# csmile-1006/ARP

Measured on AMD Instinct MI355X. Metric: frames/sec CLIP reward-labelled (256x256 ViT-B/32), higher is better.
Workload: dtype f16; 1 GPU; CLIP ViT-B/32 reward labelling, batch 1024 synthetic 256x256x3 uint8 frames per GPU resident in HBM (BASELINE.json configs[1]), random-init weights, text tower cached; parallelism=shard1 (no collective), streams_per_gpu=2

## Files before the change

### arp_amd/csrc/gemm.h

```cpp
#pragma once
#include "common.h"

#ifndef ARP_ADAMW_PIPE
#define ARP_ADAMW_PIPE 1
#endif
namespace arp {

struct GemmArgs {
    const void* A = nullptr;
    const void* W = nullptr;
    const float* bias = nullptr;
    const float* resid = nullptr;
    void* out = nullptr;
    int M = 0, N = 0, K = 0;
    int lda = 0, ldw = 0, ldr = 0, ldo = 0;
    int flags = 0;
    unsigned long long* clock_acc = nullptr;
    int ksplit = 1;
    size_t slice_stride = 0;
    const float* ln_stats = nullptr;
    const float* ln_c = nullptr;
    int ln_parts = 0;
    float ln_inv_d = 0.f, ln_eps = 0.f;
    void* xb_out = nullptr;
    int ldxb = 0;
    int m_fast = 0;
    int split3 = 0;
    float* stats_out = nullptr;
    int group_m = 0;
    int stagger_groups = 0;
    int stagger_cycles = 0;
    float alpha = 1.f;
    float out_scale = 1.f;
    const void* mask = nullptr;
    int ldm = 0;
    float* colsum_part = nullptr;
    int ovl = 0;
    float *adam_p = nullptr, *adam_m = nullptr, *adam_v = nullptr;
    void* adam_mirror = nullptr;
    int adam_mask = 0;
    unsigned int* adam_dropped = nullptr;
    float adam_gscale = 1.f, adam_lr = 0.f, adam_wd = 0.f, adam_b1 = 0.f, adam_b2 = 0.f, adam_eps = 0.f, adam_bc1 = 1.f, adam_bc2 = 1.f;
    int mix_nk16 = 0, mix_nkc_a = 0, mix_sa = 0, mix_sb = 0;
    int x8_shift = -1;
    void* dx4_out = nullptr;
    const int* mix_sptr = nullptr;
};
constexpr int GEMM_SITE_ADAMW = 26;

template <typename OutT>
inline int gemm_epilogue_refusal(const GemmArgs& g, bool fp4_side, const char* who) {
    const bool staged = ((g.N | g.ldo | g.ldr) & 3) == 0 && ((g.N | g.ldo) & (sizeof(OutT) == 1 ? 15 : 7)) == 0 && !(g.flags & 2);
    const bool fp4 = g.x8_shift >= 0 || g.dx4_out;
    const std::string w(who);
    if ((g.ln_stats || g.xb_out || g.stats_out || fp4) && !staged)
        return fail(w + ": the folded LayerNorm and the side outputs need the staged epilogue (N, ldo % 8 == 0; ldr % 4 == 0)");
    if (g.ln_stats && sizeof(OutT) != 2) return fail(w + ": the folded-LayerNorm consumer has a 16-bit output");
    if ((g.stats_out || g.split3) && sizeof(OutT) != 4) return fail(w + ": stats_out / split3 belong to the f32 epilogue");
    if (g.stats_out && g.N % 128) return fail(w + ": stats_out needs N % 128 == 0 (one (sum, sum of squares) pair per 128 columns)");
    if (fp4 && !fp4_side) return fail(w + ": the fp4 side outputs exist on the MIXC binary16-output instances only");
    if ((g.x8_shift >= 0 && !g.xb_out) || (g.split3 && !g.xb_out)) return fail(w + ": x8_shift / split3 without xb_out");
    if (g.xb_out && sizeof(OutT) != 4 && g.x8_shift < 0) return fail(w + ": xb_out of a 16-bit output is the x4 segment (x8_shift >= 0)");
    return 0;
}

constexpr int GEMM_BM = 128, GEMM_BN = 128, GEMM_THREADS = 256;
constexpr int GEMM_ROW_BYTES = 128;
constexpr int GEMM_STAGE_BYTES = (GEMM_BM + GEMM_BN) * GEMM_ROW_BYTES;
constexpr int GEMM_LDS_BYTES = 2 * GEMM_STAGE_BYTES;

__device__ __forceinline__ int xcd_remap(int bid, int nwg) {
    const int q = nwg >> 3, r = nwg & 7, xcd = bid & 7;
    const int base = (xcd < r) ? xcd * (q + 1) : r * (q + 1) + (xcd - r) * q;
    return base + (bid >> 3);
}

__device__ __forceinline__ void ln_row_stats(const GemmArgs& g, int m, float& mu, float& rs) {
    const float* st = g.ln_stats + (size_t)m * g.ln_parts * 2;
    float s = 0.f, q = 0.f;
    for (int p = 0; p < g.ln_parts; ++p) {
        s += st[2 * p];
        q += st[2 * p + 1];
    }
    mu = s * g.ln_inv_d;
    rs = 1.0f / sqrtf(fmaxf(q * g.ln_inv_d - mu * mu, 0.f) + g.ln_eps);
}
__device__ __forceinline__ float half_wave_sum(float v) {
#pragma unroll
    for (int o = 16; o > 0; o >>= 1) v += __shfl_xor(v, o, 64);
    return v;
}

template <typename T, typename OutT, int ACT, bool RESID, int SITE, int STAGES = 2>
__global__ __launch_bounds__(GEMM_THREADS) void gemm_nt_kernel(GemmArgs g) {
    extern __shared__ __attribute__((aligned(16))) char smem[];
    constexpr int EPB = GEMM_ROW_BYTES / (int)sizeof(T);
    constexpr int EPC = 16 / (int)sizeof(T);

    const int tid = threadIdx.x;
    const int lane = tid & 63;
    const int wave = __builtin_amdgcn_readfirstlane(tid >> 6);
    const int n_tiles = (g.N + GEMM_BN - 1) / GEMM_BN;
    const int m_tiles = (g.M + GEMM_BM - 1) / GEMM_BM;
    const int tile = xcd_remap(blockIdx.x, m_tiles * n_tiles);
    const int m0 = (g.m_fast ? tile % m_tiles : tile / n_tiles) * GEMM_BM;
    const int n0 = (g.m_fast ? tile / m_tiles : tile % n_tiles) * GEMM_BN;

    const T* __restrict__ A = static_cast<const T*>(g.A);
    const T* __restrict__ W = static_cast<const T*>(g.W);

    if (g.stagger_groups > 1 && blockIdx.x >= 256 && blockIdx.x < 512 && blockIdx.y == 0) {
        const unsigned long long t0 = __builtin_amdgcn_s_memtime();
        while (__builtin_amdgcn_s_memtime() - t0 < (unsigned long long)g.stagger_cycles) __builtin_amdgcn_s_sleep(64);
    }

    const int srow = lane >> 3;
    const int schunk = (lane & 7) ^ srow;
    const T* a_src[4];
    const T* w_src[4];
#pragma unroll
// ... 328 lines not shown
```

### arp_amd/csrc/gemm256.h

```cpp
#pragma once
#include <cstdlib>
#include <type_traits>

#include "common.h"
#include "gemm.h"

namespace arp {

#ifndef ARP_G2_TWO_PHASE
#define ARP_G2_TWO_PHASE 1
#endif
#ifndef ARP_G2_OVERLAP_DRAIN
#define ARP_G2_OVERLAP_DRAIN 0
#endif
constexpr int G2_BM = 256, G2_BN = 256, G2_THREADS = 512;
constexpr int G2_BUF_BYTES = (G2_BM + G2_BN) * 128;
static_assert(256 * (256 * 2 + 16) >= 2 * G2_BUF_BYTES && 256 * (256 * 2 + 16) >= 128 * (256 * 4 + 16), "epilogue tile must cover the K-tile ring");
constexpr int G2_TILE_BYTES = 256 * (256 * 2 + 16);
constexpr bool G2_MASK_SITE(int site) { return site >= 16; }
constexpr int G2_RED_OFF = G2_TILE_BYTES + 1024;
constexpr int G2_LDS_BYTES = G2_RED_OFF + 8 * 256 * 4;
constexpr int G2_B_REGION = G2_BM * 128;
constexpr int G2_GROUP_M = 8;

template <int N> __device__ __forceinline__ void wait_vmcnt() {
    if constexpr (N == 0) asm volatile("s_waitcnt vmcnt(0)" ::: "memory");
    if constexpr (N == 2) asm volatile("s_waitcnt vmcnt(2)" ::: "memory");
    if constexpr (N == 4) asm volatile("s_waitcnt vmcnt(4)" ::: "memory");
    if constexpr (N == 6) asm volatile("s_waitcnt vmcnt(6)" ::: "memory");
    if constexpr (N == 8) asm volatile("s_waitcnt vmcnt(8)" ::: "memory");
    if constexpr (N == 24) asm volatile("s_waitcnt vmcnt(24)" ::: "memory");
}
__device__ __forceinline__ void wait_units(int allow) {
    if (allow >= 3) wait_vmcnt<6>();
    else if (allow == 2) wait_vmcnt<4>();
    else if (allow == 1) wait_vmcnt<2>();
    else wait_vmcnt<0>();
}

#if defined(ARP_G2_STAMPS) || defined(ARP_G2_FINE) || defined(ARP_G2_CLOCK)
__device__ long long* arp_g2_stamps = nullptr;
#endif
#ifndef ARP_G2_MAX_VGPR
#define ARP_G2_MAX_VGPR 128
#endif
#ifndef ARP_G2_MFMA32
#define ARP_G2_MFMA32 0
#endif
#ifndef ARP_G2_MIXC_RT
#define ARP_G2_MIXC_RT 0
#endif
#ifndef ARP_G2_MIX_UNIFORM
#define ARP_G2_MIX_UNIFORM 0
#endif
#ifndef ARP_G2_ABL
#define ARP_G2_ABL 0
#endif
typedef __attribute__((ext_vector_type(16))) float f32x16_v;
template <typename T> __device__ __forceinline__ f32x16_v mfma32(u32x4_v a, u32x4_v b, f32x16_v c) {
    if constexpr (__is_same(T, f16_t))
        return __builtin_amdgcn_mfma_f32_32x32x16_f16(__builtin_bit_cast(f16x8_v, a), __builtin_bit_cast(f16x8_v, b), c, 0, 0, 0);
    else
        return __builtin_amdgcn_mfma_f32_32x32x16_bf16(__builtin_bit_cast(bf16x8_v, a), __builtin_bit_cast(bf16x8_v, b), c, 0, 0, 0);
}
template <typename T, typename OutT, int ACT, bool RESID, int SITE, bool M32 = (ARP_G2_MFMA32 != 0), int KV = ARP_G2_KV, bool MIXC = false, bool CLK = false>
__global__ __launch_bounds__(G2_THREADS, 2) __attribute__((amdgpu_num_vgpr(ARP_G2_MAX_VGPR))) void gemm256_nt_kernel(GemmArgs g) {
    extern __shared__ __attribute__((aligned(16))) char smem[];
    constexpr int EPB = 128 / (int)sizeof(T);
    constexpr int EPC = 16 / (int)sizeof(T);
    constexpr bool W32 = M32 && sizeof(T) == 2;

    const int tid = threadIdx.x;
    const int lane = tid & 63;
    const int wave = __builtin_amdgcn_readfirstlane(tid >> 6);
    const int wr = wave >> 2, wc = wave & 3;
#ifdef ARP_G2_CLOCK
    const long long clk_c0 = __builtin_amdgcn_s_memtime(), clk_r0 = __builtin_amdgcn_s_memrealtime();
#endif
    [[maybe_unused]] unsigned long long dclk_c0 = 0, dclk_r0 = 0;
    if constexpr (CLK) {
        dclk_c0 = __builtin_amdgcn_s_memtime();
        dclk_r0 = __builtin_amdgcn_s_memrealtime();
        __builtin_amdgcn_s_waitcnt(0xC07F);
    }

    const int n_tiles = (g.N + G2_BN - 1) / G2_BN;
    const int m_tiles = (g.M + G2_BM - 1) / G2_BM;
    const int total_tiles = m_tiles * n_tiles;
    const int group_m = g.group_m > 0 ? g.group_m : G2_GROUP_M;
    int m0 = 0, n0 = 0;
    auto tile_coords = [&](int tix) __attribute__((always_inline)) {
        int t = xcd_remap(tix, total_tiles);
        const int per_group = group_m * n_tiles;
        const int grp = t / per_group;
        const int first_m = grp * group_m;
        const int gsize = min(m_tiles - first_m, group_m);
// ... 189 lines not shown
    int mix_scale = 0;
    int mix_sa = g.mix_sa, mix_sb = g.mix_sb;
    if constexpr (MIXC) {
        if (g.mix_sptr) {
            mix_sa = F16C_X_SHIFT + g.mix_sptr[0];
            mix_sb = F16C_DX_SHIFT + g.mix_sptr[1];
        }
    }
    auto mfma_quadrant = [&](auto MQ, auto NQ, auto F8 = F16T{}) __attribute__((always_inline)) {
        constexpr int mq = decltype(MQ)::value, nq = decltype(NQ)::value;
        if constexpr (MIXC && sizeof(T) == 2 && !W32) {
            if constexpr (decltype(F8)::value) {
#pragma unroll
                for (int ks = 0; ks < 2; ++ks)
#pragma unroll
                    for (int ni = 0; ni < 2; ++ni)
#pragma unroll
                        for (int mi = 0; mi < 4; ++mi) acc[mq][nq][ni][mi] = mfma_fp4_scaled(breg[nq][ni][ks], areg[mi][ks], acc[mq][nq][ni][mi], mix_scale);
                return;
            }
        }
        if constexpr (W32) {
#pragma unroll
            for (int ks = 0; ks < 4; ++ks)
#pragma unroll
                for (int mi = 0; mi < 2; ++mi) acc32[mq][nq][mi] = mfma32<T>(breg[nq][0][ks], areg[mi][ks], acc32[mq][nq][mi]);
        } else {
#pragma unroll
        for (int ks = 0; ks < 2; ++ks)
#pragma unroll
            for (int ni = 0; ni < 2; ++ni)
#pragma unroll
                for (int mi = 0; mi < 4; ++mi) {
                    if constexpr (sizeof(T) == 2) {
                        acc[mq][nq][ni][mi] = mfma16<T>(breg[nq][ni][ks], areg[mi][ks], acc[mq][nq][ni][mi]);
                    } else if constexpr (sizeof(T) == 1) {
                        if (ks == 0)
                            acc[mq][nq][ni][mi] = mfma_fp8(breg[nq][ni][0], breg[nq][ni][1], areg[mi][0], areg[mi][1], acc[mq][nq][ni][mi]);
                    } else {
#pragma unroll
                        for (int j = 0; j < 4; ++j)
                            acc[mq][nq][ni][mi] = __builtin_amdgcn_mfma_f32_16x16x4f32(
                                __uint_as_float(breg[nq][ni][ks][j]), __uint_as_float(areg[mi][ks][j]), acc[mq][nq][ni][mi], 0, 0, 0);
                    }
                }
        }
    };
    auto phase_tail = [&](int ph) __attribute__((always_inline)) {
        int allow = G - 3 - ph;
        allow = allow > 3 ? 3 : allow;
        wait_units(allow);
        __builtin_amdgcn_sched_barrier(0);
        __builtin_amdgcn_s_barrier();
        __builtin_amdgcn_sched_barrier(0);
    };
    auto compute = [&](auto MQ, auto NQ) __attribute__((always_inline)) {
        __builtin_amdgcn_s_setprio(1);
        mfma_quadrant(MQ, NQ);
        __builtin_amdgcn_s_setprio(0);
        __builtin_amdgcn_sched_barrier(0);
        __builtin_amdgcn_s_barrier();
        __builtin_amdgcn_sched_barrier(0);
    };
#if ARP_G2_TWO_PHASE
    const int S2 = 2 * nk;
    auto issue_step = [&](int st) __attribute__((always_inline)) {
        const int t4 = (st >> 1) * 4;
        if (st & 1) {
            issue(t4 + 3, U3{});
        } else {
            issue(t4 + 0, U0{});
            issue(t4 + 1, U1{});
            issue(t4 + 2, U2{});
        }
    };
    auto step_cnt = [&](int st) __attribute__((always_inline)) { return st < S2 ? ((st & 1) ? 2 : 6) : 0; };
    auto wait_instr = [&](int n) __attribute__((always_inline)) {
        if (n >= 24) wait_vmcnt<24>();
        else if (n >= 8) wait_vmcnt<8>();
        else if (n >= 6) wait_vmcnt<6>();
        else if (n >= 2) wait_vmcnt<2>();
        else wait_vmcnt<0>();
    };
    int young = 0;
    auto phase_tail2 = [&](int p) __attribute__((always_inline)) {
        wait_instr(step_cnt(p + 2) + step_cnt(p + 3) + (p + 1 <= 2 ? young : 0));
        asm volatile("s_waitcnt lgkmcnt(0)" ::: "memory");
        __builtin_amdgcn_sched_barrier(0);
        __builtin_amdgcn_s_barrier();
        __builtin_amdgcn_sched_barrier(0);
    };
    auto compute2 = [&](auto MQ, auto NQA, auto NQB, auto F8 = F16T{}) __attribute__((always_inline)) {
        __builtin_amdgcn_s_setprio(1);
        mfma_quadrant(MQ, NQA, F8);
        mfma_quadrant(MQ, NQB, F8);
        __builtin_amdgcn_s_setprio(0);
        __builtin_amdgcn_sched_barrier(0);
        __builtin_amdgcn_s_barrier();
        __builtin_amdgcn_sched_barrier(0);
    };
#endif
    bool pre_issued = false;
    bool pre_issued_bias = false;
    bool pre4 = false;
    for (int tix = blockIdx.x; tix < total_tiles; tix += gridDim.x) {
#ifdef ARP_G2_STAMPS
    long long st_[6];
    st_[0] = __builtin_amdgcn_s_memtime();
#define ARP_STAMP(i) st_[i] = __builtin_amdgcn_s_memtime()
#else
#define ARP_STAMP(i)
#endif
    tile_coords(tix);
    setup_src();
    float* bias_s = reinterpret_cast<float*>(smem + G2_TILE_BYTES);
    if (g.bias && wave == 0 && !pre_issued_bias) bias_dma(n0);
    if constexpr (W32) {
#pragma unroll
        for (int a = 0; a < 2; ++a)
#pragma unroll
            for (int b = 0; b < 2; ++b)
#pragma unroll
                for (int c = 0; c < 2; ++c)
#pragma unroll
                    for (int d = 0; d < 16; ++d) acc32[a][b][c][d] = 0.f;
    } else {
#pragma unroll
    for (int a = 0; a < 2; ++a)
#pragma unroll
        for (int b = 0; b < 2; ++b)
#pragma unroll
            for (int c = 0; c < 2; ++c)
#pragma unroll
                for (int d = 0; d < 4; ++d) acc[a][b][c][d] = f32x4_v{0.f, 0.f, 0.f, 0.f};
    }
#ifdef ARP_G2_FINE
    long long f_[12];
    for (int i = 0; i < 12; ++i) f_[i] = 0;
#define ARP_FST(i) if (kt == (nk >> 1)) f_[i] = __builtin_amdgcn_s_memtime()
#else
#define ARP_FST(i)
#endif
#if ARP_G2_TWO_PHASE
    if (!pre_issued) {
        issue_step(0);
        issue_step(1);
        issue_step(2);
    }
    young = pre4 ? 16 : 0;
    wait_instr(step_cnt(1) + step_cnt(2) + young);
    __builtin_amdgcn_sched_barrier(0);
    __builtin_amdgcn_s_barrier();
    __builtin_amdgcn_sched_barrier(0);
    if (wr == 1) {
        __builtin_amdgcn_s_barrier();
    }
    __builtin_amdgcn_sched_barrier(0);

    int kt_first = 0;
    if constexpr (KV == 1 && !ARP_G2_OVERLAP_DRAIN) {
        auto tail_ss = [&]() __attribute__((always_inline)) {
            wait_vmcnt<8>();
            __builtin_amdgcn_s_waitcnt(0xC07F);
            __builtin_amdgcn_sched_barrier(0);
            __builtin_amdgcn_s_barrier();
            __builtin_amdgcn_sched_barrier(0);
        };
        auto ktile_ss = [&](int kt, auto BUF, auto F8) __attribute__((always_inline)) {
            const char* buf = smem + ((MIXC && RESID && ARP_G2_MIXC_RT) ? (kt & 1) : decltype(BUF)::value) * G2_BUF_BYTES;
            if constexpr (MIXC && decltype(F8)::value) mix_scale = 0x7f7f7f00 | (127 - (kt < g.mix_nk16 + g.mix_nkc_a ? mix_sa : mix_sb));
            load_a(buf, 0, F8);
            load_b(buf, I0{}, F8);
            load_b(buf, I1{}, F8);
            issue_ss(kt + 1, U3{});
            tail_ss();
            compute2(I0{}, I0{}, I1{}, F8);
            load_a(buf, 1, F8);
            issue_ss(kt + 2, U0{});
            issue_ss(kt + 2, U1{});
            issue_ss(kt + 2, U2{});
            tail_ss();
            compute2(I1{}, I1{}, I0{}, F8);
        };
        auto run_ss = [&](int kt_end, auto F8) __attribute__((always_inline)) {
            if (kt_first < kt_end && (kt_first & 1)) {
                ktile_ss(kt_first, I1{}, F8);
                ++kt_first;
            }
            for (; kt_first + 1 < kt_end; kt_first += 2) {
                ktile_ss(kt_first, I0{}, F8);
                ktile_ss(kt_first + 1, I1{}, F8);
            }
            if (kt_first < kt_end) {
                ktile_ss(kt_first, I0{}, F8);
                ++kt_first;
            }
        };
        if constexpr (MIXC) {
            run_ss(g.mix_nk16, F16T{});
            run_ss(nk, F8T{});
            kt_first = nk;
        } else {
            run_ss(nk - 2, F16T{});
        }
    }
    auto ktile_tail = [&](int kt, auto F8) __attribute__((always_inline)) {
        const char* buf = smem + (kt & 1) * G2_BUF_BYTES;
        const int p = 2 * kt;
        abl_kt = kt;
        if constexpr (MIXC && decltype(F8)::value) mix_scale = 0x7f7f7f00 | (127 - (kt < g.mix_nk16 + g.mix_nkc_a ? mix_sa : mix_sb));
        ARP_FST(0);
        load_a(buf, 0, F8);
        load_b(buf, I0{}, F8);
        load_b(buf, I1{}, F8);
        issue_step(p + 3);
        ARP_FST(1);
        phase_tail2(p);
        ARP_FST(2);
        compute2(I0{}, I0{}, I1{}, F8);
        ARP_FST(4);
        load_a(buf, 1, F8);
        issue_step(p + 4);
        ARP_FST(5);
        phase_tail2(p + 1);
        ARP_FST(6);
        compute2(I1{}, I1{}, I0{}, F8);
        ARP_FST(8);
    };
    if constexpr (!MIXC) {
        for (int kt = kt_first; kt < nk; ++kt) ktile_tail(kt, F16T{});
    }
    if constexpr (MIXC) wait_vmcnt<0>();
#else
    if (!pre_issued) {
        issue(0, U0{});
        issue(1, U1{});
        issue(2, U2{});
        issue(3, U3{});
        issue(4, U0{});
    }
    {
        const int last = G - 1 < 4 ? G - 1 : 4;
        wait_units(last - 1);
// ... 22 lines not shown
        issue(ph + 7, U3{});
        phase_tail(ph + 2);
        compute(I1{}, I1{});
        issue(ph + 8, U0{});
        phase_tail(ph + 3);
        compute(I1{}, I0{});
    }
#endif
    if (wr == 0) {
        __builtin_amdgcn_s_barrier();
    }
    __builtin_amdgcn_sched_barrier(0);
    if constexpr (MIXC) {
        __builtin_amdgcn_s_barrier();
        __builtin_amdgcn_sched_barrier(0);
    }
#ifdef ARP_G2_FINE
    if (arp_g2_stamps && (threadIdx.x & 63) == 0) {
        long long* d = arp_g2_stamps + ((size_t)tix * 8 + wave) * 16;
        for (int i = 0; i < 9; ++i) d[i] = f_[i];
    }
#endif

    ARP_STAMP(1);
    auto epilogue = [&]() {
    OutT* out = static_cast<OutT*>(g.out);
#ifdef ARP_G2_EXPERIMENT_SAME_TILE
    if (g.flags & 16) out -= (size_t)m0 * g.ldo + n0;
#endif
    const bool vec_ok = ((g.N | g.ldo | g.ldr) & 3) == 0;
    if (g.flags & 1) {
        float sacc = 0.f;
#pragma unroll
        for (int a = 0; a < 2; ++a)
#pragma unroll
            for (int b = 0; b < 2; ++b)
#pragma unroll
                for (int c = 0; c < NI; ++c)
#pragma unroll
                    for (int d = 0; d < MI; ++d) {
                        const f32x4_v t = acc4(a, b, c, d);
                        sacc += t[0] + t[1] + t[2] + t[3];
                    }
        if (sacc == 12345.678f) Elem<OutT>::st(out, sacc);
        return;
    }
    const bool staged = vec_ok && ((g.N | g.ldo) & (sizeof(OutT) == 1 ? 15 : 7)) == 0 && !(g.flags & 2);
    if (staged) {
        float4 bq[2][NI];
#pragma unroll
        for (int nq = 0; nq < 2; ++nq)
#pragma unroll
            for (int ni = 0; ni < NI; ++ni)
                bq[nq][ni] = g.bias ? *reinterpret_cast<const float4*>(bias_s + wc * 64 + nq * 32 + ni * CSTEP + cl) : make_float4(0.f, 0.f, 0.f, 0.f);
        if constexpr (sizeof(OutT) == 1) {
            constexpr int RS8 = 256 + 16;
#pragma unroll
            for (int mq = 0; mq < 2; ++mq)
#pragma unroll
                for (int mi = 0; mi < MI; ++mi) {
                    const int row = wr * 128 + mq * 64 + mi * RSTEP + rl;
#pragma unroll
                    for (int nq = 0; nq < 2; ++nq)
#pragma unroll
                        for (int ni = 0; ni < NI; ++ni) {
                            const int col = wc * 64 + nq * 32 + ni * CSTEP + cl;
                            const f32x4_v a4 = acc4(mq, nq, ni, mi);
                            const float4 b = bq[nq][ni];
                            float v[4] = {a4[0] * g.alpha + b.x, a4[1] * g.alpha + b.y, a4[2] * g.alpha + b.z, a4[3] * g.alpha + b.w};
#pragma unroll
                            for (int j = 0; j < 4; ++j) v[j] = apply_act<ACT, true>(v[j]) * g.out_scale;
                            *reinterpret_cast<uint32_t*>(smem + row * RS8 + col) = pack_fp8x4(v[0], v[1], v[2], v[3]);
                        }
                }
            __syncthreads();
#pragma unroll 4
            for (int it = 0; it < 8; ++it) {
                const int r = it * 32 + wave * 4 + (lane >> 4);
                const int m = m0 + r, n = n0 + (lane & 15) * 16;
                if (m < g.M && n < g.N)
                    *reinterpret_cast<u32x4_v*>(reinterpret_cast<char*>(out) + (size_t)m * g.ldo + n) = *reinterpret_cast<const u32x4_v*>(smem + r * RS8 + (lane & 15) * 16);
            }
        } else if constexpr (sizeof(OutT) == 2) {
            constexpr int RS = 256 * 2 + 16;
            auto stage16 = [&](auto LN) {
                float* lnst = reinterpret_cast<float*>(smem + G2_RED_OFF);
                float4 cq[LN.value ? 2 : 1][LN.value ? NI : 1];
                if constexpr (LN.value) {
                    if (tid < 256) {
                        const float2* st = reinterpret_cast<const float2*>(g.ln_stats + (size_t)min(m0 + tid, g.M - 1) * g.ln_parts * 2);
                        float2 pr[8];
#pragma unroll
                        for (int p = 0; p < 8; ++p) pr[p] = st[min(p, g.ln_parts - 1)];
                        float s = 0.f, q = 0.f;
#pragma unroll
                        for (int p = 0; p < 8; ++p)
                            if (p < g.ln_parts) { s += pr[p].x; q += pr[p].y; }
                        const float mu = s * g.ln_inv_d;
                        lnst[2 * tid] = mu;
                        lnst[2 * tid + 1] = 1.0f / sqrtf(fmaxf(q * g.ln_inv_d - mu * mu, 0.f) + g.ln_eps);
                    }
#pragma unroll
                    for (int nq = 0; nq < 2; ++nq)
#pragma unroll
                        for (int ni = 0; ni < NI; ++ni)
                            cq[nq][ni] = *reinterpret_cast<const float4*>(g.ln_c + min(n0 + wc * 64 + nq * 32 + ni * CSTEP + cl, g.N - 4));
                    __syncthreads();
                }
#pragma unroll
                for (int mq = 0; mq < 2; ++mq)
#pragma unroll
                    for (int mi = 0; mi < MI; ++mi) {
                        const int row = wr * 128 + mq * 64 + mi * RSTEP + rl;
                        float mu = 0.f, rs = 1.f;
                        if constexpr (LN.value) { mu = lnst[2 * row]; rs = lnst[2 * row + 1]; }
#pragma unroll
                        for (int nq = 0; nq < 2; ++nq)
#pragma unroll
                            for (int ni = 0; ni < NI; ++ni) {
                                const int col = wc * 64 + nq * 32 + ni * CSTEP + cl;
                                const f32x4_v a4 = acc4(mq, nq, ni, mi);
                                float v[4] = {a4[0], a4[1], a4[2], a4[3]};
                                if constexpr (sizeof(T) == 1) { v[0] *= g.alpha; v[1] *= g.alpha; v[2] *= g.alpha; v[3] *= g.alpha; }
                                if constexpr (LN.value) {
                                    const float4 c4 = cq[LN.value ? nq : 0][LN.value ? ni : 0];
                                    v[0] = rs * (v[0] - mu * c4.x); v[1] = rs * (v[1] - mu * c4.y);
                                    v[2] = rs * (v[2] - mu * c4.z); v[3] = rs * (v[3] - mu * c4.w);
                                }
                                if constexpr ((ARP_G2_ABL & 8) == 0) {
                                    const float4 b = bq[nq][ni];
                                    v[0] += b.x; v[1] += b.y; v[2] += b.z; v[3] += b.w;
                                    apply_act4<ACT, sizeof(T) <= 2>(v);
                                }
                                *reinterpret_cast<uint2*>(smem + row * RS + col * 2) = make_uint2(pack2<OutT>(v[0], v[1]), pack2<OutT>(v[2], v[3]));
                                if constexpr (MIXC && __is_same(OutT, f16_t)) {
                                    if (g.dx4_out && m0 + row < g.M && n0 + col < g.N) {
                                        constexpr float sdx = (float)(1 << F16C_DX_SHIFT);
                                        *reinterpret_cast<uint16_t*>(static_cast<char*>(g.dx4_out) + (size_t)(m0 + row) * g.ldxb + ((n0 + col) >> 1)) =
                                            pack_fp4x4((v[0] - h2f(f2h(v[0]))) * sdx, (v[1] - h2f(f2h(v[1]))) * sdx, (v[2] - h2f(f2h(v[2]))) * sdx, (v[3] - h2f(f2h(v[3]))) * sdx);
                                    }
                                }
                            }
                    }
            };
            if constexpr (G2_MASK_SITE(SITE)) {
                stage16(std::false_type{});
            } else {
                if (g.ln_stats) stage16(std::true_type{});
                else stage16(std::false_type{});
            }
#if ARP_G2_TWO_PHASE && ARP_G2_OVERLAP_DRAIN
            if (g.ovl && tix + (int)gridDim.x < total_tiles && m0 + G2_BM <= g.M && n0 + G2_BN <= g.N && nk >= 4) {
                asm volatile("s_waitcnt lgkmcnt(0)" ::: "memory");
                __builtin_amdgcn_sched_barrier(0);
                __builtin_amdgcn_s_barrier();
                __builtin_amdgcn_sched_barrier(0);
                u32x4_v regs[16];
#pragma unroll
                for (int it = 0; it < 16; ++it)
                    regs[it] = *reinterpret_cast<const u32x4_v*>(smem + (it * 16 + wave * 2 + (lane >> 5)) * RS + (lane & 31) * 16);
                asm volatile("s_waitcnt lgkmcnt(0)" ::: "memory");
                __builtin_amdgcn_sched_barrier(0);
                __builtin_amdgcn_s_barrier();
                __builtin_amdgcn_sched_barrier(0);
                OutT* obase = out + (size_t)(m0 + wave * 2 + (lane >> 5)) * g.ldo + n0 + (lane & 31) * 8;
                tile_coords(tix + gridDim.x);
                setup_src();
                if (g.bias && wave == 0) bias_dma(n0);
                issue_step(0);
                issue_step(1);
                issue_step(2);
                __builtin_amdgcn_sched_barrier(0);
#pragma unroll
                for (int it = 0; it < 16; ++it) *reinterpret_cast<u32x4_v*>(obase + (size_t)it * 16 * g.ldo) = regs[it];
                __builtin_amdgcn_sched_barrier(0);
                pre_issued = pre_issued_bias = pre4 = true;
                return;
            }
#endif
            ARP_STAMP(2);
            __syncthreads();
            ARP_STAMP(3);
            if (G2_MASK_SITE(SITE) && g.mask) {
                const OutT* __restrict__ mk = static_cast<const OutT*>(g.mask);
                float colacc[8] = {0.f, 0.f, 0.f, 0.f, 0.f, 0.f, 0.f, 0.f};
#pragma unroll 4
                for (int it = 0; it < 16; ++it) {
                    const int r = it * 16 + wave * 2 + (lane >> 5);
                    const int m = m0 + r, n = n0 + (lane & 31) * 8;
                    if (m < g.M && n < g.N) {
                        u32x4_v v = *reinterpret_cast<const u32x4_v*>(smem + r * RS + (lane & 31) * 16);
                        const u32x4_v mv = *reinterpret_cast<const u32x4_v*>(mk + (size_t)m * g.ldm + n);
#pragma unroll
                        for (int w = 0; w < 4; ++w) {
                            const uint32_t mag = mv[w] & 0x7fff7fffu;
                            const uint32_t nz = ((mag & 0xffffu) ? 0xffffu : 0u) | ((mag >> 16) ? 0xffff0000u : 0u);
                            const uint32_t pos = ((mv[w] & 0x8000u) ? 0u : 0xffffu) | ((mv[w] & 0x80000000u) ? 0u : 0xffff0000u);
                            const uint32_t kept = v[w] & nz & pos;
                            v[w] = kept;
                            OutT pr[2];
                            memcpy(pr, &kept, 4);
                            colacc[2 * w] += Elem<OutT>::ld(&pr[0]);
                            colacc[2 * w + 1] += Elem<OutT>::ld(&pr[1]);
                        }
                        *reinterpret_cast<u32x4_v*>(out + (size_t)m * g.ldo + n) = v;
                    }
                }
                if (g.colsum_part) {
                    float* red = reinterpret_cast<float*>(smem + G2_RED_OFF);
#pragma unroll
                    for (int e = 0; e < 8; ++e) colacc[e] += __shfl_xor(colacc[e], 32, 64);
                    if (lane < 32) {
#pragma unroll
                        for (int e = 0; e < 8; ++e) red[wave * 256 + lane * 8 + e] = colacc[e];
                    }
                    __syncthreads();
                    if (tid < 256 && n0 + tid < g.N) {
                        float t = 0.f;
#pragma unroll
                        for (int w = 0; w < 8; ++w) t += red[w * 256 + tid];
                        g.colsum_part[(size_t)(m0 / G2_BM) * g.N + n0 + tid] = t;
                    }
                }
                return;
            }
#pragma unroll 4
            for (int it = 0; it < 16; ++it) {
                const int r = it * 16 + wave * 2 + (lane >> 5);
                const int m = m0 + r, n = n0 + (lane & 31) * 8;
                if (m < g.M && n < g.N) {
                    const u32x4_v v = *reinterpret_cast<const u32x4_v*>(smem + r * RS + (lane & 31) * 16);
                    if (g.flags & 4) __builtin_nontemporal_store(v, reinterpret_cast<u32x4_v*>(out + (size_t)m * g.ldo + n));
                    else *reinterpret_cast<u32x4_v*>(out + (size_t)m * g.ldo + n) = v;
                    if constexpr (MIXC && __is_same(OutT, f16_t)) {
                        if (g.x8_shift >= 0) {
                            const float inv = 1.0f / (float)(1 << g.x8_shift);
                            const uint32_t e0 = v[0], e1 = v[1], e2 = v[2], e3 = v[3];
                            uint32_t w4 = 0;
                            w4 = __builtin_amdgcn_cvt_scalef32_pk_fp4_f16(w4, __builtin_bit_cast(f16x2_v, e0), inv, 0);
                            w4 = __builtin_amdgcn_cvt_scalef32_pk_fp4_f16(w4, __builtin_bit_cast(f16x2_v, e1), inv, 1);
                            w4 = __builtin_amdgcn_cvt_scalef32_pk_fp4_f16(w4, __builtin_bit_cast(f16x2_v, e2), inv, 2);
                            w4 = __builtin_amdgcn_cvt_scalef32_pk_fp4_f16(w4, __builtin_bit_cast(f16x2_v, e3), inv, 3);
                            *reinterpret_cast<uint32_t*>(static_cast<char*>(g.xb_out) + (size_t)m * g.ldxb + (n >> 1)) = w4;
                        }
                    }
                }
            }
        } else {
            constexpr int RSF = 256 * 4 + 16;
#ifndef ARP_G2_RES_EARLY
#define ARP_G2_RES_EARLY 1
#endif
            float4 rres[2][16];
            auto load_res = [&](int p) {
                if constexpr (RESID) {
#pragma unroll
                    for (int it = 0; it < 16; ++it) {
                        const int lr = it * 8 + wave;
                        const int m = m0 + (lr >> 6) * 128 + p * 64 + (lr & 63), n = n0 + lane * 4;
                        if constexpr ((ARP_G2_ABL & 4) == 0) rres[p][it] = *reinterpret_cast<const float4*>(g.resid + (size_t)min(m, g.M - 1) * g.ldr + min(n, g.N - 4));
                        else rres[p][it] = make_float4(0.f, 0.f, 0.f, 0.f);
                    }
// ... 17 lines not shown
                            if constexpr (sizeof(T) == 1) { v[0] *= g.alpha; v[1] *= g.alpha; v[2] *= g.alpha; v[3] *= g.alpha; }
                            const float4 b = bq[nq][ni];
                            v[0] += b.x; v[1] += b.y; v[2] += b.z; v[3] += b.w;
#pragma unroll
                            for (int j = 0; j < 4; ++j) v[j] = apply_act<ACT, sizeof(T) <= 2>(v[j]);
                            *reinterpret_cast<float4*>(smem + lrow * RSF + col * 4) = make_float4(v[0], v[1], v[2], v[3]);
                        }
                __syncthreads();
                if (p == 0 && ARP_G2_RES_EARLY) load_res(1);
#pragma unroll
                for (int it = 0; it < 16; ++it) {
                    const int lr = it * 8 + wave;
                    const int m = m0 + (lr >> 6) * 128 + p * 64 + (lr & 63), n = n0 + lane * 4;
                    const bool ok = m < g.M && n < g.N;
                    float4 v = make_float4(0.f, 0.f, 0.f, 0.f);
                    if (ok) {
                        v = *reinterpret_cast<const float4*>(smem + lr * RSF + lane * 16);
                        if constexpr (RESID) {
                            const float4 r = rres[p][it];
                            v.x += r.x; v.y += r.y; v.z += r.z; v.w += r.w;
                        }
                        if (g.out) *reinterpret_cast<float4*>(reinterpret_cast<float*>(out) + (size_t)m * g.ldo + n) = v;
                        if (g.xb_out) {
                            if (g.split3) store_split3(static_cast<T*>(g.xb_out) + (size_t)m * g.ldxb + n, (size_t)g.N, v.x, v.y, v.z, v.w);
                            else store4(static_cast<T*>(g.xb_out) + (size_t)m * g.ldxb + n, v.x, v.y, v.z, v.w);
                        }
                    }
                    if (g.stats_out) {
                        const float s = half_wave_sum((v.x + v.y) + (v.z + v.w));
                        const float q = half_wave_sum((v.x * v.x + v.y * v.y) + (v.z * v.z + v.w * v.w));
                        if ((lane & 31) == 0 && ok) {
                            float* st = g.stats_out + ((size_t)m * (g.N >> 7) + ((n0 >> 7) + (lane >> 5))) * 2;
                            st[0] = s;
                            st[1] = q;
                        }
                    }
                }
            }
        }
        return;
    }
#pragma unroll
    for (int mq = 0; mq < 2; ++mq)
#pragma unroll
        for (int mi = 0; mi < MI; ++mi) {
            const int m = m0 + wr * 128 + mq * 64 + mi * RSTEP + rl;
            if (m >= g.M) continue;
#pragma unroll
            for (int nq = 0; nq < 2; ++nq)
#pragma unroll
                for (int ni = 0; ni < NI; ++ni) {
                    const int n = n0 + wc * 64 + nq * 32 + ni * CSTEP + cl;
                    if (n >= g.N) continue;
                    const f32x4_v a4 = acc4(mq, nq, ni, mi);
                    float v[4] = {a4[0], a4[1], a4[2], a4[3]};
                    if constexpr (sizeof(T) == 1) { v[0] *= g.alpha; v[1] *= g.alpha; v[2] *= g.alpha; v[3] *= g.alpha; }
                    if (vec_ok) {
                        if (g.bias) {
                            const float4 b = *reinterpret_cast<const float4*>(g.bias + n);
                            v[0] += b.x; v[1] += b.y; v[2] += b.z; v[3] += b.w;
                        }
#pragma unroll
                        for (int j = 0; j < 4; ++j) v[j] = apply_act<ACT, sizeof(T) <= 2>(v[j]);
                        if constexpr (RESID) {
                            const float4 r = *reinterpret_cast<const float4*>(g.resid + (size_t)m * g.ldr + n);
                            v[0] += r.x; v[1] += r.y; v[2] += r.z; v[3] += r.w;
                        }
                        store4(out + (size_t)m * g.ldo + n, v[0], v[1], v[2], v[3]);
                    } else {
#pragma unroll
                        for (int j = 0; j < 4; ++j) {
                            if (n + j >= g.N) break;
                            float x = v[j] + (g.bias ? g.bias[n + j] : 0.f);
                            x = apply_act<ACT, sizeof(T) <= 2>(x);
                            if constexpr (RESID) x += g.resid[(size_t)m * g.ldr + n + j];
                            Elem<OutT>::st(out + (size_t)m * g.ldo + n + j, x);
                        }
                    }
                }
        }
    };
    pre_issued = false;
    pre_issued_bias = false;
    pre4 = false;
    epilogue();
#ifdef ARP_G2_STAMPS
    ARP_STAMP(4);
    asm volatile("s_waitcnt vmcnt(0)" ::: "memory");
    ARP_STAMP(5);
    if (arp_g2_stamps && (threadIdx.x & 63) == 0) {
        long long* d = arp_g2_stamps + ((size_t)tix * 8 + wave) * 8;
        for (int i = 0; i < 6; ++i) d[i] = st_[i];
    }
#endif
    if (!pre_issued && tix + (int)gridDim.x < total_tiles) {
        __syncthreads();
        tile_coords(tix + gridDim.x);
        setup_src();
        if (g.bias && wave == 0) bias_dma(n0);
        pre_issued_bias = true;
#if ARP_G2_TWO_PHASE
        issue_step(0);
        issue_step(1);
        issue_step(2);
#else
        issue(0, U0{});
        issue(1, U1{});
        issue(2, U2{});
        issue(3, U3{});
        issue(4, U0{});
#endif
        pre_issued = true;
    }
    if constexpr (MIXC) break;
    }
#ifdef ARP_G2_CLOCK
    if (arp_g2_stamps && threadIdx.x == 0) {
        arp_g2_stamps[blockIdx.x * 2] = __builtin_amdgcn_s_memtime() - clk_c0;
        arp_g2_stamps[blockIdx.x * 2 + 1] = __builtin_amdgcn_s_memrealtime() - clk_r0;
    }
#endif
    if constexpr (CLK) {
        const unsigned long long c1 = __builtin_amdgcn_s_memtime(), r1 = __builtin_amdgcn_s_memrealtime();
        if (g.clock_acc && threadIdx.x == 0) {
            atomicAdd(g.clock_acc, c1 - dclk_c0);
            atomicAdd(g.clock_acc + 1, r1 - dclk_r0);
            atomicAdd(g.clock_acc + 2, 1ull);
        }
    }
}

template <typename T, typename OutT, int ACT, bool RESID, int SITE, bool M32 = (ARP_G2_MFMA32 != 0), int KV = ARP_G2_KV, bool MIXC = false, bool CLK = false>
inline int launch_gemm256_nt(const GemmArgs& g, hipStream_t stream) {
    constexpr int EPB = 128 / (int)sizeof(T);
    if (g.M <= 0) return 0;
    if (g.N <= 0 || g.K % EPB != 0 || g.K <= 0 || g.lda % (16 / (int)sizeof(T)) != 0 || g.ldw % (16 / (int)sizeof(T)) != 0)
        return fail("gemm256_nt: unsupported shape M=" + std::to_string(g.M) + " N=" + std::to_string(g.N) +
                    " K=" + std::to_string(g.K));
    if (int rc = gemm_epilogue_refusal<OutT>(g, MIXC && __is_same(OutT, f16_t), "gemm256_nt")) return rc;
    if (g.ln_stats && G2_MASK_SITE(SITE)) return fail("gemm256_nt: no folded-LayerNorm epilogue in the masked-epilogue instances");
    if (g.ln_stats && (g.ln_parts < 1 || g.ln_parts > 8)) return fail("gemm256_nt: the folded-LayerNorm epilogue holds at most 8 partial sums per row (width <= 1024)");
    if (g.mask && (!G2_MASK_SITE(SITE) || sizeof(OutT) != 2 || ((g.N | g.ldo | g.ldm | g.ldr) & 7) || (g.flags & 3)))
        return fail("gemm256_nt: the masked epilogue needs a 16-bit output and N, ldo, ldm multiples of 8");
    if (KV == 1 && ((size_t)G2_BM * g.lda * sizeof(T) >= (1ull << 32) || (size_t)G2_BN * g.ldw * sizeof(T) >= (1ull << 32)))
        return fail("gemm256_nt: row stride too large for the 32-bit tile offsets of the KV = 1 K loop");
    if (MIXC && (sizeof(T) != 2 || g.mix_nk16 <= 0 || 64 * (g.mix_nk16 + g.mix_nkc_a) > g.K || g.K / 64 - g.mix_nk16 < 2 || !KV || (ARP_G2_MIX_UNIFORM && (g.N % G2_BN || !(g.flags & 32))) || g.mix_sa < 0 || g.mix_sa > 120 || g.mix_sb < 0 || g.mix_sb > 120))
        return fail("gemm256_nt: bad mixed binary16 / e2m1 K-tile plan (needs >= 2 trailing fp4 K-tiles, i.e. Kc >= 512 with one correction segment)");
    auto kern = gemm256_nt_kernel<T, OutT, ACT, RESID, SITE, M32, KV, MIXC, CLK>;
    static bool attr_set = false;
    if (!attr_set) {
        ARP_HIP_OK(hipFuncSetAttribute(reinterpret_cast<const void*>(kern), hipFuncAttributeMaxDynamicSharedMemorySize,
                                       G2_LDS_BYTES));
        attr_set = true;
    }
    const int m_tiles = (g.M + G2_BM - 1) / G2_BM;
    const int n_tiles = (g.N + G2_BN - 1) / G2_BN;
    int grid = m_tiles * n_tiles;
    static int persist = -1, n_cu = 0;
    if (persist < 0) {
        const char* e = getenv("ARP_GEMM_PERSIST");
        persist = e ? atoi(e) : 0;
        int dev = 0;
        hipDeviceProp_t prop;
        if (hipGetDevice(&dev) == hipSuccess && hipGetDeviceProperties(&prop, dev) == hipSuccess) n_cu = prop.multiProcessorCount;
        if (n_cu <= 0 || (n_cu & 7)) n_cu = 256;
    }
    if (!MIXC && persist && grid > n_cu) grid = n_cu;
    static int tpw = -1;
    if (tpw < 0) {
        const char* e = getenv("ARP_GEMM_TPW");
        tpw = e ? atoi(e) : 1;
        if (tpw < 1) tpw = 1;
    }
    GemmArgs ga = g;
    static int group_env = -1;
    if (group_env < 0) {
        const char* e = getenv("ARP_GEMM_GROUP_M");
        group_env = e ? atoi(e) : 0;
    }
    if (group_env > 0 && ga.group_m == 0) ga.group_m = group_env;
#if ARP_G2_OVERLAP_DRAIN
    if (!MIXC && sizeof(OutT) == 2 && tpw > 1 && !persist && grid >= 2 * n_cu) {
        grid = (grid + tpw - 1) / tpw;
        ga.ovl = 1;
    }
    if (!MIXC && sizeof(OutT) == 2 && persist) ga.ovl = 1;
#endif
    hipLaunchKernelGGL(kern, dim3(grid), dim3(G2_THREADS), G2_LDS_BYTES, stream, ga);
    ARP_HIP_OK(hipGetLastError());
    return 0;
}

}
#include "gemm2w.h"
namespace arp {

template <typename T, typename OutT, int ACT, bool RESID, int SITE>
inline int launch_gemm_auto(const GemmArgs& g, hipStream_t stream, int force = 0) {
    const long tiles256 = (long)((g.M + G2_BM - 1) / G2_BM) * ((g.N + G2_BN - 1) / G2_BN);
    if constexpr (sizeof(T) == 2) {
        if (force == 3 && gemm2w_has(__is_same(T, bf16_t) ? 1 : 2, sizeof(OutT) == 4 ? 1 : 0, ACT, RESID ? 1 : 0) && g.K % 64 == 0 && !(g.N & 7) &&
            !(g.ldo & 7) && !(RESID && (g.ldr & 3)) && !g.ln_stats && !g.stats_out && !g.xb_out && g.ksplit <= 1 && g.alpha == 1.f)
            return launch_gemm2w<T, OutT, ACT, RESID>(g, stream);
    }
    if (g.alpha != 1.f) return launch_gemm_nt<T, OutT, ACT, RESID, SITE>(g, stream);
    if (force == 1) return launch_gemm_nt<T, OutT, ACT, RESID, SITE>(g, stream);
    if (force == 2 || tiles256 >= 192) {
        static const bool splitm = [] { const char* e = getenv("ARP_GEMM_SPLITM"); return e && atoi(e) != 0; }();
        const int n_t = (g.N + G2_BN - 1) / G2_BN, m_t = (g.M + G2_BM - 1) / G2_BM;
        const long rounds = tiles256 / 256, rem_tiles = tiles256 - rounds * 256;
        const int full_m = (int)(rounds * 256 / n_t);
        if (splitm && rounds >= 1 && rounds <= 3 && rem_tiles > 8 && rem_tiles <= 128 && full_m < m_t && g.ksplit <= 1 && !g.ln_stats && !g.stats_out && !g.xb_out &&
            !g.mask && !g.colsum_part && !g.adam_p && !(g.flags & 3) && g.mix_nk16 == 0) {
            GemmArgs a = g, b = g;
            a.M = full_m * G2_BM;
            b.M = g.M - a.M;
            b.A = static_cast<const T*>(g.A) + (size_t)a.M * g.lda;
            b.out = static_cast<OutT*>(g.out) + (size_t)a.M * g.ldo;
            if (g.resid) b.resid = g.resid + (size_t)a.M * g.ldr;
            if (int rc = launch_gemm256_nt<T, OutT, ACT, RESID, SITE>(a, stream)) return rc;
            return launch_gemm_nt<T, OutT, ACT, RESID, SITE>(b, stream);
        }
        return launch_gemm256_nt<T, OutT, ACT, RESID, SITE>(g, stream);
    }
    return launch_gemm_nt<T, OutT, ACT, RESID, SITE>(g, stream);
}

}
```

### arp_amd/csrc/qkvattn.hip

```cpp
#include "qkvattn.h"

#include <cstdlib>

#include "attention.h"
#include "gemm.h"
#include "gemm256.h"
#include "kloop192.h"

namespace arp {

constexpr int QA_THREADS = 512;
constexpr int QA_BUF_BYTES = K192_BUF_BYTES;
constexpr int QA_KV_ROWS = 320;
constexpr int QA_K_OFF = 256 * 128;
constexpr int QA_V_OFF = QA_K_OFF + QA_KV_ROWS * 128;
static_assert(QA_V_OFF + QA_KV_ROWS * 128 <= 2 * QA_BUF_BYTES, "q/k/v images must fit the K-tile ring");
constexpr int QA_LDS_BYTES = 2 * QA_BUF_BYTES + 192 * 4;

#ifdef ARP_QA_STAMPS
__device__ long long* arp_qa_stamps = nullptr;
#define QA_STAMP(i) st_[i] = __builtin_amdgcn_s_memtime()
#else
#define QA_STAMP(i)
#endif

template <typename T>
__global__ __launch_bounds__(QA_THREADS, 2) void qkv_attn_kernel(QkvAttnArgs g) {
    static_assert(sizeof(T) == 2, "16-bit operand types only");
    extern __shared__ __attribute__((aligned(16))) char smem[];
    constexpr int EPB = 64, EPC = 8;
    constexpr int NT = 4;

    const int tid = threadIdx.x;
    const int lane = tid & 63;
    const int wave = __builtin_amdgcn_readfirstlane(tid >> 6);
    const int wr = wave >> 2, wc = wave & 3;

    const int m_tiles = (g.B + g.fpt - 1) / g.fpt;
    const int n_tiles = g.heads;
    int mt, head;
    {
        int t = xcd_remap(blockIdx.x, m_tiles * n_tiles);
        const int group_m = g.group_m > 0 ? g.group_m : G2_GROUP_M;
        const int per_group = group_m * n_tiles;
        const int grp = t / per_group;
        const int first_m = grp * group_m;
        const int gsize = min(m_tiles - first_m, group_m);
        t -= grp * per_group;
        mt = first_m + t % gsize;
        head = t / gsize;
    }
    const int f0 = mt * g.fpt;
    const int nf = min(g.fpt, g.B - f0);
    const int m0 = f0 * g.N;
    const int rows = nf * g.N;
    const int Mtot = g.B * g.N;
    const int n0 = head * 192;

    const T* __restrict__ A = static_cast<const T*>(g.A);
    const T* __restrict__ W = static_cast<const T*>(g.W);

#ifdef ARP_QA_STAMPS
    long long st_[5];
#endif
    QA_STAMP(0);
    f32x4_v acc[2][3][4];
    kloop_256x192<T>(smem, A, W, g.bias, g.lda, g.ldw, m0, n0, Mtot, g.heads * 192, g.K, acc);
    QA_STAMP(1);
    const int fr = lane & 15, fg = lane >> 4;
    float* bias_s = reinterpret_cast<float*>(smem + K192_RING_BYTES);

    for (int i = tid; i < 2 * 64 * 8; i += QA_THREADS) {
        const int img = i >> 9, rr = (i >> 3) & 63, ch = i & 7;
        *reinterpret_cast<u32x4_v*>(smem + (img ? QA_V_OFF : QA_K_OFF) + (256 + rr) * 128 + ch * 16) = u32x4_v{0u, 0u, 0u, 0u};
    }
#pragma unroll
    for (int mq = 0; mq < 2; ++mq)
#pragma unroll
        for (int mi = 0; mi < 4; ++mi) {
            const int row = wr * 128 + mq * 64 + mi * 16 + fr;
#pragma unroll
            for (int ni = 0; ni < 3; ++ni) {
                const int col = wc * 48 + ni * 16 + fg * 4;
                const int img = col >> 6, d = col & 63;
                const float4 b = *reinterpret_cast<const float4*>(bias_s + col);
                const f32x4_v a4 = acc[mq][ni][mi];
                const int off = (img == 0 ? 0 : (img == 1 ? QA_K_OFF : QA_V_OFF)) + row * 128 + (((d >> 3) ^ (row & 7)) << 4) + (d & 7) * 2;
                *reinterpret_cast<uint2*>(smem + off) = make_uint2(pack2<T>(a4[0] + b.x, a4[1] + b.y), pack2<T>(a4[2] + b.z, a4[3] + b.w));
            }
        }
    __syncthreads();
    QA_STAMP(2);

    const char* Ks = smem + QA_K_OFF;
    const char* Vs = smem + QA_V_OFF;
    const int N = g.N;
    const int nqb = (g.nq + 15) >> 4;
    const float c2 = g.scale * 1.4426950408889634f;
    const int trq = fr >> 2, trp = fr & 3;
    for (int u = wave; u < nf * nqb; u += 8) {
        const int f = u / nqb, qb = u - f * nqb;
        const int R0 = f * N;
        const int qidx = qb * 16 + fr;
        const bool qvalid = qidx < N;
        const int qabs = R0 + (qvalid ? qidx : N - 1);
        u32x4_v qf[2];
#pragma unroll
        for (int ks = 0; ks < 2; ++ks) qf[ks] = *reinterpret_cast<const u32x4_v*>(smem + qabs * 128 + (((ks * 4 + fg) ^ (qabs & 7)) << 4));
        f32x4_v s[NT];
#pragma unroll
        for (int kt = 0; kt < NT; ++kt) {
            s[kt] = f32x4_v{0.f, 0.f, 0.f, 0.f};
            const int krow = R0 + kt * 16 + fr;
#pragma unroll
            for (int ks = 0; ks < 2; ++ks) {
                const u32x4_v kf = *reinterpret_cast<const u32x4_v*>(Ks + krow * 128 + (((ks * 4 + fg) ^ (krow & 7)) << 4));
                s[kt] = mfma16<T>(kf, qf[ks], s[kt]);
            }
        }
        const int klim = g.causal ? (qidx < N ? qidx + 1 : N) : N;
        float mx = -INFINITY;
        if (!g.causal) {
#pragma unroll
            for (int kt = 0; kt < NT; ++kt)
#pragma unroll
                for (int r = 0; r < 4; ++r) {
                    if (kt * 16 + 15 >= N) {
                        const int key = kt * 16 + fg * 4 + r;
                        s[kt][r] = (key < N) ? s[kt][r] : -INFINITY;
                    }
                    mx = fmaxf(mx, s[kt][r]);
                }
        } else {
#pragma unroll
        for (int kt = 0; kt < NT; ++kt)
#pragma unroll
            for (int r = 0; r < 4; ++r) {
                const int key = kt * 16 + fg * 4 + r;
                const float v = (key < klim) ? s[kt][r] : -INFINITY;
                s[kt][r] = v;
                mx = fmaxf(mx, v);
            }
        }
        mx = fmaxf(mx, __shfl_xor(mx, 16, 64));
        mx = fmaxf(mx, __shfl_xor(mx, 32, 64));
        const float mc = mx * c2;
        float sum = 0.f;
#pragma unroll
        for (int kt = 0; kt < NT; ++kt)
#pragma unroll
            for (int r = 0; r < 4; ++r) {
                const float p = __builtin_amdgcn_exp2f(fmaf(s[kt][r], c2, -mc));
                s[kt][r] = p;
                sum += p;
            }
        sum += __shfl_xor(sum, 16, 64);
        sum += __shfl_xor(sum, 32, 64);
        const float inv = 1.0f / sum;

        f32x4_v o[4];
#pragma unroll
        for (int dt = 0; dt < 4; ++dt) o[dt] = f32x4_v{0.f, 0.f, 0.f, 0.f};
#pragma unroll
        for (int st = 0; st < NT / 2; ++st) {
            u32x4_v pb;
            pb[0] = pack2<T>(s[2 * st][0], s[2 * st][1]);
            pb[1] = pack2<T>(s[2 * st][2], s[2 * st][3]);
            pb[2] = pack2<T>(s[2 * st + 1][0], s[2 * st + 1][1]);
            pb[3] = pack2<T>(s[2 * st + 1][2], s[2 * st + 1][3]);
            const int k0 = R0 + 32 * st + 4 * fg + trq, k1 = k0 + 16;
#pragma unroll
            for (int dt = 0; dt < 4; ++dt) {
                const int ch = 2 * dt + (trp >> 1);
                const tr_b64_v lo = __builtin_amdgcn_ds_read_tr16_b64_v4i16(
                    (__attribute__((address_space(3))) tr_b64_v*)(Vs + k0 * 128 + ((ch ^ (k0 & 7)) << 4) + (trp & 1) * 8));
                const tr_b64_v hi = __builtin_amdgcn_ds_read_tr16_b64_v4i16(
                    (__attribute__((address_space(3))) tr_b64_v*)(Vs + k1 * 128 + ((ch ^ (k1 & 7)) << 4) + (trp & 1) * 8));
                const u32x2_v l2 = __builtin_bit_cast(u32x2_v, lo), h2 = __builtin_bit_cast(u32x2_v, hi);
                const u32x4_v va = {l2[0], l2[1], h2[0], h2[1]};
                o[dt] = mfma16<T>(va, pb, o[dt]);
            }
        }
        if (qvalid && qidx < g.nq) {
            const int row = R0 + qidx;
#pragma unroll
            for (int dt = 0; dt < 4; ++dt) {
                const int d = dt * 16 + fg * 4;
                *reinterpret_cast<uint2*>(smem + row * 128 + (((d >> 3) ^ (row & 7)) << 4) + (d & 7) * 2) =
                    make_uint2(pack2<T>(o[dt][0] * inv, o[dt][1] * inv), pack2<T>(o[dt][2] * inv, o[dt][3] * inv));
            }
        }
    }
    QA_STAMP(3);
    __syncthreads();
    T* out = static_cast<T*>(g.out);
#pragma unroll
    for (int it = 0; it < 4; ++it) {
        const int row = it * 64 + (tid >> 3), ch = tid & 7;
        if (row < rows && (row % N) < g.nq) {
            const u32x4_v v = *reinterpret_cast<const u32x4_v*>(smem + row * 128 + ((ch ^ (row & 7)) << 4));
            *reinterpret_cast<u32x4_v*>(out + (size_t)(m0 + row) * g.ldo + head * 64 + ch * 8) = v;
        }
    }
#ifdef ARP_QA_STAMPS
    asm volatile("s_waitcnt vmcnt(0)" ::: "memory");
    QA_STAMP(4);
    if (arp_qa_stamps && lane == 0) {
        long long* d = arp_qa_stamps + ((size_t)blockIdx.x * 8 + wave) * 8;
        for (int i = 0; i < 5; ++i) d[i] = st_[i];
    }
#endif
}

template <typename T>
static int launch_qkv_attn_impl(QkvAttnArgs g, hipStream_t stream) {
    if (g.B <= 0) return 0;
    if (!qkv_attn_supported(g.N, g.heads * 64, g.heads, (int)sizeof(T)) || g.K % 64 != 0 || g.lda % 8 != 0 || g.ldw % 8 != 0 || g.ldo % 8 != 0)
        return fail("qkv_attn: unsupported shape N=" + std::to_string(g.N) + " heads=" + std::to_string(g.heads) + " K=" + std::to_string(g.K));
    g.fpt = 256 / g.N;
    if (g.nq <= 0 || g.nq > g.N) g.nq = g.N;
    g.scale = 1.0f / sqrtf(64.0f);
    auto kern = qkv_attn_kernel<T>;
    static bool attr_set = false;
    if (!attr_set) {
        ARP_HIP_OK(hipFuncSetAttribute(reinterpret_cast<const void*>(kern), hipFuncAttributeMaxDynamicSharedMemorySize, QA_LDS_BYTES));
        attr_set = true;
    }
    const int m_tiles = (g.B + g.fpt - 1) / g.fpt;
    hipLaunchKernelGGL(kern, dim3(m_tiles * g.heads), dim3(QA_THREADS), QA_LDS_BYTES, stream, g);
    ARP_HIP_OK(hipGetLastError());
    return 0;
}


int launch_qkv_attn_f16(QkvAttnArgs g, hipStream_t stream) { return launch_qkv_attn_impl<f16_t>(g, stream); }
int launch_qkv_attn_bf16(QkvAttnArgs g, hipStream_t stream) { return launch_qkv_attn_impl<bf16_t>(g, stream); }

}
```

Before: 102,000 frames/s.

## Use per-wave epilogue staging in GEMM and per-wave output stores in attention

```diff
diff --git a/arp_amd/csrc/gemm.h b/arp_amd/csrc/gemm.h
--- a/arp_amd/csrc/gemm.h
+++ b/arp_amd/csrc/gemm.h
@@ -35,7 +35,6 @@
     const void* mask = nullptr;
     int ldm = 0;
     float* colsum_part = nullptr;
-    int ovl = 0;
     float *adam_p = nullptr, *adam_m = nullptr, *adam_v = nullptr;
     void* adam_mirror = nullptr;
     int adam_mask = 0;
diff --git a/arp_amd/csrc/gemm256.h b/arp_amd/csrc/gemm256.h
--- a/arp_amd/csrc/gemm256.h
+++ b/arp_amd/csrc/gemm256.h
@@ -9,9 +9,6 @@
 
 #ifndef ARP_G2_TWO_PHASE
 #define ARP_G2_TWO_PHASE 1
-#endif
-#ifndef ARP_G2_OVERLAP_DRAIN
-#define ARP_G2_OVERLAP_DRAIN 0
 #endif
 constexpr int G2_BM = 256, G2_BN = 256, G2_THREADS = 512;
 constexpr int G2_BUF_BYTES = (G2_BM + G2_BN) * 128;
@@ -367,9 +364,8 @@
         else if (n >= 2) wait_vmcnt<2>();
         else wait_vmcnt<0>();
     };
-    int young = 0;
     auto phase_tail2 = [&](int p) __attribute__((always_inline)) {
-        wait_instr(step_cnt(p + 2) + step_cnt(p + 3) + (p + 1 <= 2 ? young : 0));
+        wait_instr(step_cnt(p + 2) + step_cnt(p + 3));
         asm volatile("s_waitcnt lgkmcnt(0)" ::: "memory");
         __builtin_amdgcn_sched_barrier(0);
         __builtin_amdgcn_s_barrier();
@@ -387,7 +383,6 @@
 #endif
     bool pre_issued = false;
     bool pre_issued_bias = false;
-    bool pre4 = false;
     for (int tix = blockIdx.x; tix < total_tiles; tix += gridDim.x) {
 #ifdef ARP_G2_STAMPS
     long long st_[6];
@@ -432,8 +427,7 @@
         issue_step(1);
         issue_step(2);
     }
-    young = pre4 ? 16 : 0;
-    wait_instr(step_cnt(1) + step_cnt(2) + young);
+    wait_instr(step_cnt(1) + step_cnt(2));
     __builtin_amdgcn_sched_barrier(0);
     __builtin_amdgcn_s_barrier();
     __builtin_amdgcn_sched_barrier(0);
@@ -443,7 +437,7 @@
     __builtin_amdgcn_sched_barrier(0);
 
     int kt_first = 0;
-    if constexpr (KV == 1 && !ARP_G2_OVERLAP_DRAIN) {
+    if constexpr (KV == 1) {
         auto tail_ss = [&]() __attribute__((always_inline)) {
             wait_vmcnt<8>();
             __builtin_amdgcn_s_waitcnt(0xC07F);
@@ -632,6 +626,61 @@
                     *reinterpret_cast<u32x4_v*>(reinterpret_cast<char*>(out) + (size_t)m * g.ldo + n) = *reinterpret_cast<const u32x4_v*>(smem + r * RS8 + (lane & 15) * 16);
             }
         } else if constexpr (sizeof(OutT) == 2) {
+            if constexpr (!G2_MASK_SITE(SITE) && !MIXC) {
+                if (!g.ln_stats) {
+                    int ln;
+                    asm volatile("v_mbcnt_lo_u32_b32 %0, -1, 0\n\tv_mbcnt_hi_u32_b32 %0, -1, %0" : "=v"(ln));
+                    const int rl_e = W32 ? (ln & 31) : (ln & 15), cl_e = (W32 ? (ln >> 5) : (ln >> 4)) * 4;
+                    char* reg = smem + wave * (64 * 128);
+                    const int key = (rl_e >> 1) & 7;
+                    char* wbase = reg + rl_e * 128 + (cl_e & 7) * 2;
+                    const int kk = ((cl_e >> 3) ^ key) << 4;
+                    const int rrow = ln >> 3, rch = ln & 7;
+                    const char* rbase = reg + rrow * 128;
+                    const int rk0 = (rch ^ (rrow >> 1)) << 4, rk1 = (rch ^ (rrow >> 1) ^ 4) << 4;
+                    const int mrow = m0 + wr * 128 + rrow;
+                    const bool ncol_ok = n0 + wc * 64 + rch * 8 < g.N;
+                    OutT* obase = out + (size_t)mrow * g.ldo + (n0 + wc * 64 + rch * 8);
+                    const bool nt = g.flags & 4;
+#pragma unroll
+                    for (int mq = 0; mq < 2; ++mq) {
+#pragma unroll
+                        for (int mi = 0; mi < MI; ++mi)
+#pragma unroll
+                            for (int nq = 0; nq < 2; ++nq)
+#pragma unroll
+                                for (int ni = 0; ni < NI; ++ni) {
+                                    const f32x4_v a4 = acc4(mq, nq, ni, mi);
+                                    float v[4] = {a4[0], a4[1], a4[2], a4[3]};
+                                    if constexpr (sizeof(T) == 1) { v[0] *= g.alpha; v[1] *= g.alpha; v[2] *= g.alpha; v[3] *= g.alpha; }
+                                    if constexpr ((ARP_G2_ABL & 8) == 0) {
+                                        const float4 b = bq[nq][ni];
+                                        v[0] += b.x; v[1] += b.y; v[2] += b.z; v[3] += b.w;
+                                        apply_act4<ACT, sizeof(T) <= 2>(v);
+                                    }
+                                    *reinterpret_cast<uint2*>(wbase + mi * RSTEP * 128 + ((((nq * 32 + ni * CSTEP) >> 3) << 4) ^ kk)) =
+                                        make_uint2(pack2<OutT>(v[0], v[1]), pack2<OutT>(v[2], v[3]));
+                                }
+                        if (mq) ARP_STAMP(3);
+                        asm volatile("s_waitcnt lgkmcnt(0)" ::: "memory");
+                        u32x4_v sv[8];
+#pragma unroll
+                        for (int it = 0; it < 8; ++it) sv[it] = *reinterpret_cast<const u32x4_v*>(rbase + it * 8 * 128 + ((it & 1) ? rk1 : rk0));
+#pragma unroll
+                        for (int it = 0; it < 8; ++it) {
+                            const int r = mq * 64 + it * 8;
+                            if (ncol_ok && mrow + r < g.M) {
+                                u32x4_v* dp = reinterpret_cast<u32x4_v*>(obase + (size_t)r * g.ldo);
+                                if (nt) __builtin_nontemporal_store(sv[it], dp);
+                                else *dp = sv[it];
+                            }
+                        }
+                        __builtin_amdgcn_sched_barrier(0);
+                        if (!mq) ARP_STAMP(2);
+                    }
+                    return;
+                }
+            }
             constexpr int RS = 256 * 2 + 16;
             auto stage16 = [&](auto LN) {
                 float* lnst = reinterpret_cast<float*>(smem + G2_RED_OFF);
@@ -699,35 +748,6 @@
                 if (g.ln_stats) stage16(std::true_type{});
                 else stage16(std::false_type{});
             }
-#if ARP_G2_TWO_PHASE && ARP_G2_OVERLAP_DRAIN
-            if (g.ovl && tix + (int)gridDim.x < total_tiles && m0 + G2_BM <= g.M && n0 + G2_BN <= g.N && nk >= 4) {
-                asm volatile("s_waitcnt lgkmcnt(0)" ::: "memory");
-                __builtin_amdgcn_sched_barrier(0);
-                __builtin_amdgcn_s_barrier();
-                __builtin_amdgcn_sched_barrier(0);
-                u32x4_v regs[16];
-#pragma unroll
-                for (int it = 0; it < 16; ++it)
-                    regs[it] = *reinterpret_cast<const u32x4_v*>(smem + (it * 16 + wave * 2 + (lane >> 5)) * RS + (lane & 31) * 16);
-                asm volatile("s_waitcnt lgkmcnt(0)" ::: "memory");
-                __builtin_amdgcn_sched_barrier(0);
-                __builtin_amdgcn_s_barrier();
-                __builtin_amdgcn_sched_barrier(0);
-                OutT* obase = out + (size_t)(m0 + wave * 2 + (lane >> 5)) * g.ldo + n0 + (lane & 31) * 8;
-                tile_coords(tix + gridDim.x);
-                setup_src();
-                if (g.bias && wave == 0) bias_dma(n0);
-                issue_step(0);
-                issue_step(1);
-                issue_step(2);
-                __builtin_amdgcn_sched_barrier(0);
-#pragma unroll
-                for (int it = 0; it < 16; ++it) *reinterpret_cast<u32x4_v*>(obase + (size_t)it * 16 * g.ldo) = regs[it];
-                __builtin_amdgcn_sched_barrier(0);
-                pre_issued = pre_issued_bias = pre4 = true;
-                return;
-            }
-#endif
             ARP_STAMP(2);
             __syncthreads();
             ARP_STAMP(3);
@@ -911,7 +931,6 @@
     };
     pre_issued = false;
     pre_issued_bias = false;
-    pre4 = false;
     epilogue();
 #ifdef ARP_G2_STAMPS
     ARP_STAMP(4);
@@ -1008,13 +1027,7 @@
         group_env = e ? atoi(e) : 0;
     }
     if (group_env > 0 && ga.group_m == 0) ga.group_m = group_env;
-#if ARP_G2_OVERLAP_DRAIN
-    if (!MIXC && sizeof(OutT) == 2 && tpw > 1 && !persist && grid >= 2 * n_cu) {
-        grid = (grid + tpw - 1) / tpw;
-        ga.ovl = 1;
-    }
-    if (!MIXC && sizeof(OutT) == 2 && persist) ga.ovl = 1;
-#endif
+    if (!MIXC && sizeof(OutT) == 2 && tpw > 1 && !persist) grid = (grid + tpw - 1) / tpw;
     hipLaunchKernelGGL(kern, dim3(grid), dim3(G2_THREADS), G2_LDS_BYTES, stream, ga);
     ARP_HIP_OK(hipGetLastError());
     return 0;
diff --git a/arp_amd/csrc/qkvattn.hip b/arp_amd/csrc/qkvattn.hip
--- a/arp_amd/csrc/qkvattn.hip
+++ b/arp_amd/csrc/qkvattn.hip
@@ -98,6 +98,7 @@
     const int nqb = (g.nq + 15) >> 4;
     const float c2 = g.scale * 1.4426950408889634f;
     const int trq = fr >> 2, trp = fr & 3;
+    T* out = static_cast<T*>(g.out);
     for (int u = wave; u < nf * nqb; u += 8) {
         const int f = u / nqb, qb = u - f * nqb;
         const int R0 = f * N;
@@ -190,18 +191,18 @@
                     make_uint2(pack2<T>(o[dt][0] * inv, o[dt][1] * inv), pack2<T>(o[dt][2] * inv, o[dt][3] * inv));
             }
         }
+        asm volatile("s_waitcnt lgkmcnt(0)" ::: "memory");
+#pragma unroll
+        for (int it = 0; it < 2; ++it) {
+            const int qi = qb * 16 + it * 8 + (lane >> 3), ch = lane & 7;
+            const int row = R0 + qi;
+            if (qi < N && qi < g.nq && row < rows) {
+                const u32x4_v v = *reinterpret_cast<const u32x4_v*>(smem + row * 128 + ((ch ^ (row & 7)) << 4));
+                *reinterpret_cast<u32x4_v*>(out + (size_t)(m0 + row) * g.ldo + head * 64 + ch * 8) = v;
+            }
+        }
     }
     QA_STAMP(3);
-    __syncthreads();
-    T* out = static_cast<T*>(g.out);
-#pragma unroll
-    for (int it = 0; it < 4; ++it) {
-        const int row = it * 64 + (tid >> 3), ch = tid & 7;
-        if (row < rows && (row % N) < g.nq) {
-            const u32x4_v v = *reinterpret_cast<const u32x4_v*>(smem + row * 128 + ((ch ^ (row & 7)) << 4));
-            *reinterpret_cast<u32x4_v*>(out + (size_t)(m0 + row) * g.ldo + head * 64 + ch * 8) = v;
-        }
-    }
 #ifdef ARP_QA_STAMPS
     asm volatile("s_waitcnt vmcnt(0)" ::: "memory");
     QA_STAMP(4);
```

Result: no change. 102,800 frames/s, median of 6 (+0.8%).
